# omuses/hqp

Hardware: AMD Instinct MI355X
Metric: KKT factor+solve/sec (fp64) (higher is better)
Workload: dtype f64; 1 GPU; C4 = BASELINE configs[3], the metric's 10^6-variable DOCP: multistage LQ optimal control QP, K=200 stages, nx=5000 states, nu=50 controls -> n=1015000 me=1005000 m=20000, dense fx/fu handed over as blocks, x_0 fixed, box bounds on u; plugin LQDOCP (STAGED engine), one system per GPU; stages=200, nx=5000, nu=50, n=1015000, me=1005000, m=20000, plugin=LQDOCP, kkt_dim_full=2040000

## Files before the change

### hqp_amd/csrc/hqpkkt.hip

```cpp
#include "hqpkkt_handle.hpp"

char g_last_hip_error[512] = "";
std::atomic<long long> g_live_bufs[2];

namespace kktdev {
__global__ void k_mfma_selftest(const double *A, const double *B, double *C) {
  const int lane = threadIdx.x & 63, lr = lane & 15, lk = lane >> 4;
  double4_t acc = {0.0, 0.0, 0.0, 0.0};
  for (int k0 = 0; k0 < 16; k0 += 4)
    acc = mfma_f64(A[lr * 16 + k0 + lk], B[(k0 + lk) * 16 + lr], acc);
  for (int rg = 0; rg < 4; rg++) C[(lk + 4 * rg) * 16 + lr] = acc[rg];
}
}

int hqpkkt_default_opts(hqpkkt_opts *o) {
  if (!o) return HQPKKT_E_NULL;
  std::memset(o, 0, sizeof(*o));
  o->mode = HQPKKT_MODE_FULL;
  o->device = 0;
  o->loc = HQPKKT_LOC_HOST;
  o->tol = 1.0;
  o->eps = 1e-10;
  o->pivot_eps = 1e-20;
  o->leaf_size = 0;
// ... 603 lines not shown
    case HQPKKT_E_SING: return "matrix is singular";
    case HQPKKT_E_FORMAT: return "CSR input not sorted / out of range";
    case HQPKKT_E_NULL: return "NULL objects passed";
    case HQPKKT_E_RANGE: return "parameter out of range";
    case HQPKKT_E_INTERN: return "call order violated";
    case HQPKKT_E_DEVICE: return g_last_hip_error[0] ? g_last_hip_error : "HIP device error";
    default: return "unknown status";
  }
}


int hqpkkt_debug_get(const hqpkkt_t *h, int what, int *out, long long *len) {
  if (!h || !len) return HQPKKT_E_NULL;
  if (!h->analyzed && what != 40) return HQPKKT_E_INTERN;
  const Analysis &an = h->an;
  const std::vector<int> *v = nullptr;
  std::vector<int> tmp;
  switch (what) {
    case 0: v = &an.q2e; break;
    case 1: v = &an.piv_start; break;
    case 2: v = &an.npiv; break;
    case 3: v = &an.nbor; break;
    case 4: v = &an.parent; break;
    case 5: v = &an.level; break;
    case 6:
      tmp.assign(an.bptr.begin(), an.bptr.end());
      v = &tmp;
      break;
    case 7: v = &an.bidx; break;
    case 8: v = &an.ent_er; break;
    case 9: v = &an.ent_ec; break;
    case 10: v = &an.node_owner; break;
    case 11: v = &an.xroots; break;
    case 20: case 21: case 22: case 23: case 24: case 25: case 26: case 27: case 28: case 32: case 33: case 34: case 35: case 36: case 37: case 38: case 39: case 41: case 42: case 43: case 44: case 45: case 46: case 47: {
      const int e = staged_debug_get(h, what, tmp);
      if (e) return e;
      v = &tmp;
      break;
    }
    case 30:
      tmp = {h->zd_used, h->zd_weak ? 1 : 0};
      v = &tmp;
      break;
    case 31:
      tmp = {h->top_n, h->top_n ? h->top_lt : h->an.nlevels, (int)h->top_lds, h->top_ns, h->small_tree ? 1 : 0, h->tree_factor ? 1 : 0, h->top_split ? 1 : 0};
      v = &tmp;
      break;
    case 40:
      tmp = {(int)g_live_bufs[0].load(), (int)g_live_bufs[1].load()};
      v = &tmp;
      break;
    default: return HQPKKT_E_RANGE;
  }
  *len = (long long)v->size();
  if (out && !v->empty()) std::memcpy(out, v->data(), sizeof(int) * v->size());
  return 0;
}

#ifdef HQPKKT_STAMPS
extern "C" int hqpkkt_debug_stamps(hqpkkt_t *h, int *out) {
  HIPCHK(hipDeviceSynchronize());
  HIPCHK(hipMemcpy(out, h->td.flags.p, sizeof(int) * 64, hipMemcpyDeviceToHost));
  return 0;
}
#endif

int hqpkkt_debug_read(hqpkkt_t *h, int what, int node, double *out, long long cap, long long *len) {
// ... 61 lines not shown
```

### hqp_amd/csrc/staged.hip.h

```cpp
#pragma once
#include <hip/hip_runtime.h>

#include <algorithm>

#include "staged_plan.hpp"
#include "staged_gemm.hip.h"

namespace stg {

struct HTerm {
  int s1, s2, wi;
};
__global__ void k_st_add_h(int nent, const long long *__restrict__ dst, const int *__restrict__ tptr,
                           const HTerm *__restrict__ terms, const double *__restrict__ vals,
                           const double *__restrict__ wt, double *__restrict__ G, int add) {
  const int e = blockIdx.x * blockDim.x + threadIdx.x;
  if (e >= nent) return;
  double s = 0.0;
  for (int k = tptr[e]; k < tptr[e + 1]; k++) s += vals[terms[k].s1] * vals[terms[k].s2] * wt[terms[k].wi];
  if (add)
    G[dst[e]] += s;
  else
    G[dst[e]] = s;
}
// ... 1647 lines not shown
};
__global__ void __launch_bounds__(256) k_st_fwd_small(FwdSmall a) {
  extern __shared__ __attribute__((aligned(16))) double sm[];
  const int tid = threadIdx.x, nt = blockDim.x;
  const int r = a.dyn[0], nl = a.dyn[1];
  const int *Rl = a.dyn + 2, *Ll = a.dyn + 2 + a.capn;
  const double *uy = a.uy;
  double *yN = sm;
  for (int i = tid; i < a.m; i += nt) a.u[i] = uy[i];
  for (int s = tid; s < r; s += nt) {
    double v = uy[a.m + s];
    for (int li = 0; li < nl; li++) v -= a.t[(long long)li * a.ldt + s] * a.eta[li];
    yN[Rl[s]] = v;
  }
  for (int li = tid; li < nl; li += nt) yN[Ll[li]] = a.eta[li];
  __syncthreads();
  const int c = r + nl;
  for (int i = tid; i < a.e; i += nt) a.dy[a.eq_rows[i]] = yN[i];
  for (int i = tid; i < a.cap_next; i += nt) a.eta_next[i] = (a.e + i < c) ? yN[a.e + i] : 0.0;
}

__global__ void k_st_x0_fixed(int n0, const int *__restrict__ fix_rows, const int *__restrict__ fix_src,
                              const double *__restrict__ vals, const double *__restrict__ r2, double *__restrict__ x0,
                              double *__restrict__ eta0, int cap0) {
  const int i = blockIdx.x * blockDim.x + threadIdx.x;
  if (i < n0) x0[i] = -r2[fix_rows[i]] / vals[fix_src[i]];
  if (i < cap0) eta0[i] = 0.0;
}
__global__ void k_st_y_fixed(int n0, const int *__restrict__ fix_rows, const int *__restrict__ fix_src,
                             const double *__restrict__ vals, const double *__restrict__ tmp, double *__restrict__ dy) {
  const int i = blockIdx.x * blockDim.x + threadIdx.x;
  if (i < n0) dy[fix_rows[i]] = -tmp[i] / vals[fix_src[i]];
}
__device__ void x0_lu_solve(const double *__restrict__ LU, long long ldq, const double *__restrict__ perm, int qmax, int q,
                            double *t, double *T) {
  const int tid = threadIdx.x, lane = tid & 63, wave = tid >> 6, nw = blockDim.x >> 6;
  if (tid == 0)
    for (int s = 0; s < q; s++) {
      const int r = (int)perm[qmax + s];
      const double x = t[s];
      t[s] = t[r], t[r] = x;
    }
  __syncthreads();
  for (int b0 = 0; b0 < q; b0 += 64) {
    const int nb = min(64, q - b0);
    for (int i = wave; i < nb; i += nw) {
      double sum = 0.0;
      for (int j = lane; j < b0; j += 64) sum += LU[(long long)(b0 + i) * ldq + j] * t[j];
      sum = kktdev::wave_sum(sum);
      if (lane == 0) t[b0 + i] -= sum;
    }
    for (int e = tid; e < nb * nb; e += blockDim.x) T[(e / nb) * 65 + e % nb] = LU[(long long)(b0 + e / nb) * ldq + b0 + e % nb];
    __syncthreads();
    if (wave == 0) {
      double y = lane < nb ? t[b0 + lane] : 0.0;
      for (int s = 0; s < nb; s++) {
        const double ys = __shfl(y, s);
        if (lane > s && lane < nb) y -= T[lane * 65 + s] * ys;
      }
      if (lane < nb) t[b0 + lane] = y;
    }
    __syncthreads();
  }
  for (int b0 = ((q - 1) / 64) * 64; b0 >= 0; b0 -= 64) {
    const int nb = min(64, q - b0);
    for (int i = wave; i < nb; i += nw) {
// ... 242 lines not shown
```

### hqp_amd/csrc/staged_engine.hip

```cpp
#include "hqpkkt_handle.hpp"

#include <algorithm>
#include <limits>

#include "staged.hip.h"
#include "staged_sparse.hip.h"
#include "staged_profile.hip.h"
#include "staged_rows.hip.h"
#include "staged_hess.hip.h"
#include "staged_host.hip.h"

static void staged_hess_symv(hqpkkt_t *h, StagedDev &d, const double *x, double *y) {
  const kktdev::StagedPlan &P = d.plan;
  if (d.hs_nz_max > 0 || !P.hess_packed) {
    const int nzmax = std::max(d.hs_nz_max, 1);
    KLAUNCH(h, KC_RESIDUAL, stg::k_hs_symv<<<dim3(std::min((nzmax + 3) / 4, 1024), P.K + 1), 256, 0, h->stream>>>(d.hess_desc.p, d.Qd.p, x, y));
  }
  if (d.hp_chunks_max > 0) {
    KLAUNCH(h, KC_RESIDUAL, stg::k_hp_symv_tiles<<<dim3(d.hp_chunks_max, P.K + 1), 256, 0, h->stream>>>(d.hp_desc.p, d.Qd.p, x, d.hess_scr.p));
    KLAUNCH(h, KC_RESIDUAL, stg::k_hp_symv_finish<<<dim3(d.hp_nt_max, P.K + 1), stg::HP_T, 0, h->stream>>>(d.hp_desc.p, d.hess_scr.p, y));
  }
}
int staged_dense_products(hqpkkt_t *h, const Vecs &v, const double **x1, const double **x2, int *ndyn, const double **xq) {
  StagedDev &d = *h->sd;
// ... 129 lines not shown
          for (long long c : {P.h_kept[k], P.h_cut[k]}) out.push_back((int)(unsigned)(c & 0xffffffffLL)), out.push_back((int)(c >> 32));
      }
      break;
    case 44:
      out.assign(P.K + 2, 0);
      if (h->sd->ctl.p) {
        unsigned w[3] = {0, 0, 0};
        if (hipDeviceSynchronize() != hipSuccess || hipMemcpy(w, h->sd->ctl.p, sizeof(w), hipMemcpyDeviceToHost) != hipSuccess) return HQPKKT_E_DEVICE;
        out[0] = (int)(w[1] + (w[2] ? 1 : 0));
      }
      for (size_t k = 0; k < h->sd->ctrl_rows.size() && k + 1 < out.size(); k++) out[k + 1] = h->sd->ctrl_rows[k];
      break;
    case 45:
      for (int k = 0; k <= P.K && P.hess_dense; k++) {
        out.push_back(P.hess_order(k)), out.push_back(P.ldQ[k]);
        out.push_back((int)(unsigned)(P.h_kept[k] & 0xffffffffLL)), out.push_back((int)(P.h_kept[k] >> 32));
      }
      break;
    case 47:
      for (int k = 0; k <= P.K && P.hess_packed; k++) {
        const int nz = P.hess_order(k);
        const bool pk = P.stage_packed(k);
        const long long nt = (nz + P.HESS_T - 1) / P.HESS_T, tiles = pk ? P.hess_tiles(nz) : 0;
        out.push_back(pk ? P.HESS_T : 0), out.push_back((int)tiles);
        for (long long c : {pk ? tiles * P.HESS_T * P.HESS_T : (long long)nz * P.ldQ[k], P.hess_handover(nz, pk), pk ? P.hess_slots(nt) * P.HESS_T : 0LL})
          out.push_back((int)(unsigned)(c & 0xffffffffLL)), out.push_back((int)(c >> 32));
      }
      break;
    case 46:
      if (!P.wr_rows.empty()) {
        out.push_back(P.rows_vec() ? 1 : 0), out.push_back((int)P.wr_rows.size());
        for (long long c : {P.c_kept, P.c_cut}) out.push_back((int)(unsigned)(c & 0xffffffffLL)), out.push_back((int)(c >> 32));
      }
      break;
    case 38:
      for (const GemmCache::Entry &t : h->sd->gemms.entries) {
        if (!t.s.cut()) continue;
        const int row[3] = {(int)t.s.f.tiles, (int)t.s.nslab, t.s.f.kind + (t.s.seg ? 100 : 0)};
        size_t q = 0;
        while (q < out.size() && !std::equal(row, row + 3, out.begin() + q)) q += 5;
        if (q == out.size()) out.insert(out.end(), {row[0], row[1], row[2], t.s.list, 0});
        out[q + 4] += t.hits;
      }
      break;
    default: return HQPKKT_E_RANGE;
  }
  return 0;
}

extern "C" {

int hqpkkt_set_dynamics_form(hqpkkt_t *h, int form) {
  return guarded([&]() -> int {
    if (!h) return HQPKKT_E_NULL;
    if (h->opts.mode != HQPKKT_MODE_STAGED) return HQPKKT_E_INTERN;
    if (form != HQPKKT_DYN_DENSE && form != HQPKKT_DYN_SPARSE && form != HQPKKT_DYN_PROFILE) return HQPKKT_E_RANGE;
    if (!h->sd) h->sd.reset(new StagedDev);
    h->sd->plan.want_sparse = form == HQPKKT_DYN_SPARSE;
    h->sd->plan.want_profile = form == HQPKKT_DYN_PROFILE;
    return 0;
  });
}

int hqpkkt_set_dense_columns(hqpkkt_t *h, int min_entries) {
  return guarded([&]() -> int {
    if (!h) return HQPKKT_E_NULL;
// ... 383 lines not shown
      KLAUNCH(h, KC_ASSEMBLE, stg::k_hu_update<<<dim3((unsigned)units_max, (unsigned)K1), 256, 0, h->stream>>>(d.hu_desc.p, d.Qd.p, V));
      HIPCHK(hipGetLastError());
      if (h->opts.loc != HQPKKT_LOC_DEVICE) HIPCHK(hipStreamSynchronize(h->stream));
    }
    if ((int)d.hess_set.size() != K1) d.hess_set.assign(K1, 0);
    for (int k = 0; k < K1; k++)
      if (hd[k].mode == 0) d.hess_set[k] = 1;
    h->factored = false;
    return 0;
  });
}

int hqpkkt_debug_stage_ranks(hqpkkt_t *h, int *out, int cap) {
  if (!h || !out) return HQPKKT_E_NULL;
  if (!h->sd || !h->uploaded) return HQPKKT_E_INTERN;
  HIPCHK(hipSetDevice(h->opts.device));
  HIPCHK(hipStreamSynchronize(h->stream));
  const kktdev::StagedPlan &P = h->sd->plan;
  for (int k = 0; k <= P.K && 2 * k + 1 < cap; k++)
    HIPCHK(hipMemcpy(out + 2 * k, h->sd->dyn.p + P.dyn_off[k], 2 * sizeof(int), hipMemcpyDeviceToHost));
  return 0;
}

int hqpkkt_debug_stage_block(hqpkkt_t *h, int k, double *out, long long cap, long long *len) {
  if (!h || !len) return HQPKKT_E_NULL;
  if (!h->sd || !h->uploaded || h->sd->plan.sharded) return HQPKKT_E_INTERN;
  const kktdev::StagedPlan &P = h->sd->plan;
  if (k < 0 || k > P.K) return HQPKKT_E_RANGE;
  const long long n = P.nk[k];
  *len = n * n;
  if (!out) return 0;
  if (cap < n * n) return HQPKKT_E_SIZES;
  HIPCHK(hipSetDevice(h->opts.device));
  HIPCHK(hipStreamSynchronize(h->stream));
  if (n) HIPCHK(hipMemcpy2D(out, sizeof(double) * n, h->sd->V.p + P.oV[k], sizeof(double) * P.ldv[k], sizeof(double) * n, n, hipMemcpyDeviceToHost));
  return 0;
}

namespace {
__global__ void k_fill_rand(double *p, long long n, unsigned long long seed) {
  long long i = (long long)blockIdx.x * blockDim.x + threadIdx.x;
  if (i >= n) return;
  unsigned long long x = (unsigned long long)i * 0x9E3779B97F4A7C15ULL + seed;
  x ^= x >> 30, x *= 0xBF58476D1CE4E5B9ULL, x ^= x >> 27, x *= 0x94D049BB133111EBULL, x ^= x >> 31;
  p[i] = (double)(x >> 11) * (1.0 / 9007199254740992.0) - 0.5;
}
__global__ void k_gemm_check(stg::GemmArgs g, int nsample, double *err) {
  const int sidx = blockIdx.x * blockDim.x + threadIdx.x;
  if (sidx >= nsample) return;
  unsigned long long x = (unsigned long long)sidx * 0x9E3779B97F4A7C15ULL + 12345;
  x ^= x >> 29, x *= 0xBF58476D1CE4E5B9ULL, x ^= x >> 32;
  int i = (int)(x % (unsigned long long)g.M), j = (int)((x >> 20) % (unsigned long long)g.N);
  int ci = i, cj = j;
  if (g.lower && i < j) {
    const int t = i;
    i = j, j = t;
    if (!g.mirror) ci = i, cj = j;
  }
  double s = 0.0, sa = 0.0;
  for (int k = 0; k < g.K; k++) {
    const double a = g.A[(long long)k * g.lda + i], b = g.B[(long long)k * g.ldb + j];
    s += a * b, sa += fabs(a * b);
  }
  for (int k = 0; k < g.K2; k++) {
    const double a = g.A2[(long long)k * g.lda2 + i], b = g.B2[(long long)k * g.ldb2 + j];
    s += a * b, sa += fabs(a * b);
// ... 778 lines not shown
```

### hqp_amd/csrc/staged_host.hip.h

```cpp
#pragma once

struct GemmCache {
  struct Entry {
    stg::GemmRequest rq;
    stg::GemmSchedule s;
    DBuf<stg::SkUnit> units;
    DBuf<int> order;
    int hits = 0;
  };
  std::vector<Entry> entries;
  Entry *find(const stg::GemmRequest &rq) {
    for (Entry &e : entries)
      if (e.rq == rq) return &e;
    return nullptr;
  }
  int get(const stg::GemmCaps &caps, const stg::GemmRequest &rq, bool create, Entry &local, Entry *&out) {
    if ((out = find(rq))) return 0;
    if (stg::gemm_schedule(caps, rq, local.s) != stg::GEMM_SCHED_OK) return HQPKKT_E_INTERN;
    out = &local;
    if (!local.s.kept()) return 0;
    if (!create) return HQPKKT_E_INTERN;
    local.rq = rq;
    if ((!local.s.tab.units.empty() && local.units.upload(local.s.tab.units)) || (!local.s.order.empty() && local.order.upload(local.s.order))) return HQPKKT_E_MEM;
    entries.push_back(std::move(local));
// ... 38 lines not shown
  DBuf<stg::StripTab> wtabs;
  DBuf<stg::RectTab> rtabs;
  DBuf<int> gtile;
  DBuf<unsigned> gowned;
  std::vector<long long> gowned_off;
  DBuf<stg::PackRect> prects;
  std::vector<int> prect_ptr;
  DBuf<stg::DynLoc> dyn_loc;
  DBuf<double> dyn_sum;
  long long dyn_sum_x2 = 0;
  StreamOwner stream_x;
  EventOwner ev_x1, ev_w[3], ev_x[3];
  struct SymvGroup {
    int first, count, tiles, fins;
    int kfirst, klast;
  };
  DBuf<stg::SymvItem> symv_items[2];
  std::vector<SymvGroup> symv_groups[2];
  std::vector<int> symv_rows_stage[2];
  DBuf<double> zeros;
  stg::GemmCaps caps;
  GemmCache gemms;
  DBuf<double> ks_ws2;
  DBuf<double> sk_ws;
  DBuf<unsigned> sk_cnt;
  StreamOwner stream2;
  EventOwner ev_fork, ev_join;
  bool overlap = false;
  int overlap_mode = 0;
  std::vector<char> fused;
  DBuf<double> fv_nrm;
  DBuf<unsigned> ctl;
  std::vector<char> ctrl_rows;
  DBuf<int> pf_rng;
  DBuf<double> pf_part;
  DBuf<stg::PackPanel> pk_tab;
  DBuf<double> pk_part;
  size_t lds_small = 0, lds_small_big = 0, lds_init = 0, lds_x0 = 0;
};

namespace {

bool env_no_symv() { static const bool v = getenv("HQPKKT_NO_SYMV") != nullptr; return v; }
int env_symv_from() { static const int v = getenv("HQPKKT_SYMV_FROM") ? atoi(getenv("HQPKKT_SYMV_FROM")) : 2048; return v; }
double env_block_gj_tol() { static const double v = getenv("HQPKKT_BLOCK_GJ_TOL") ? atof(getenv("HQPKKT_BLOCK_GJ_TOL")) : 1e-6; return v; }
bool env_spd_test_fail() { static const bool v = getenv("HQPKKT_SPD_TEST_FAIL") != nullptr; return v; }
struct StreamGuard {
  hqpkkt_t *h;
  hipStream_t s;
  ~StreamGuard() { h->stream = s; }
};
int stream_after(hqpkkt_t *h, hipEvent_t ev, hipStream_t from, hipStream_t to) {
  if (h->listing || from == to) return 0;
  HIPCHK(hipEventRecord(ev, from));
  HIPCHK(hipStreamWaitEvent(to, ev, 0));
  return 0;
}
struct StreamFork {
  hqpkkt_t *h;
  hipStream_t a, b;
  hipEvent_t ev_fork, ev_join;
  bool forked = false;
  int fork() {
    if (int e = stream_after(h, ev_fork, a, b)) return e;
    forked = true;
    return 0;
  }
  int join() {
    forked = false;
    return stream_after(h, ev_join, b, a);
  }
  ~StreamFork() {
    if (forked) (void)join();
  }
};

struct StagePtr {
  double *F, *V, *Y, *Rm, *Kinv, *Kmat, *N, *BT, *T, *v, *beta, *eta, *rho;
  int *dyn;
// ... 264 lines not shown
static void st_bwd_small(hqpkkt_t *h, StagedDev &d, int k, const StagePtr &sp, const StagePtr &sn, const double *r2, const double *gam) {
  const kktdev::StagedPlan &P = d.plan;
  stg::BwdSmall ba{P.nk[k], P.mk[k], P.nk[k + 1], P.eq_ptr[k + 1] - P.eq_ptr[k], P.capn[k], P.cap[k], P.qmax[k], d.eq_rows.p + P.eq_ptr[k], r2,
                   P.cap[k + 1] > 0 ? sn.dyn + 1 : nullptr, sn.beta, sn.BT, P.ldb[k + 1], r2 + P.nks[k], gam, sp.Kinv, sp.Kmat, P.ldq[k], sp.T, P.ldt[k],
                   sp.dyn, sp.rho, sp.beta};
  KLAUNCH(h, KC_ST_SMALL, stg::k_st_bwd_small<<<1, 256, sizeof(double) * (P.capn[k] + 3 * P.qmax[k] + 4 + 256), h->stream>>>(ba));
}
static int st_initial_state(hqpkkt_t *h, StagedDev &d, const double *r2) {
  const kktdev::StagedPlan &P = d.plan;
  hipStream_t s = h->stream;
  double *M = d.misc.p, *S = M + P.oS;
  const StagePtr s0 = stage_ptr(d, 0);
  const int n0 = P.nk[0];
  if (P.fixed_x0) {
    KLAUNCH(h, KC_ST_VEC, stg::k_st_x0_fixed<<<nblk(std::max(n0, P.cap[0])), 256, 0, s>>>(n0, d.fix_rows.p, d.fix_src.p, h->td.vals.p, r2, S,
                                                                                       s0.eta, P.cap[0]));
    return 0;
  }
  if (P.big0) {
    const int q = P.q0max, l8 = (q + 7) / 8 * 8;
    double *vec = M + P.oK0s + 3 * (long long)q + 8, *nb = vec, *pb = vec + l8, *y = vec + 2 * l8, *r = vec + 3 * l8;
    const stg::X0Vec xv{n0, P.cap[0], q, s0.dyn, M + P.oK0s, s0.v, s0.beta, nb, pb, pb, S, s0.eta};
    int e;
    KLAUNCH(h, KC_ST_VEC, stg::k_x0_rhs<<<nblk(q), 256, 0, s>>>(xv));
    if ((e = st_gemv_rows(h, stg::GemvRows{M + P.oK0, P.ldq0, q, q, nb, nullptr, nullptr, 0, nullptr, nullptr, y, 1.0})) ||
        (e = st_gemv_rows(h, stg::GemvRows{M + P.oK0m, P.ldq0, q, q, y, pb, nullptr, 0, nullptr, nullptr, r, -1.0})) ||
        (e = st_gemv_rows(h, stg::GemvRows{M + P.oK0, P.ldq0, q, q, r, y, nullptr, 0, nullptr, nullptr, pb, 1.0})))
      return e;
    KLAUNCH(h, KC_ST_VEC, stg::k_x0_out<<<nblk(n0 + P.cap[0]), 256, 0, s>>>(xv));
  }
  KLAUNCH(h, KC_ST_SMALL, stg::k_st_x0_free<<<1, 256, d.lds_x0, s>>>(n0, P.cap[0], P.q0max, M + P.oK0, M + P.oK0m, M + P.oK0s, P.ldq0, s0.dyn, s0.v,
                                                            s0.beta, S, s0.eta));
  return 0;
}
static void st_fwd_small(hqpkkt_t *h, StagedDev &d, int k, const StagePtr &sp, const StagePtr &sn, double *dy) {
  const kktdev::StagedPlan &P = d.plan;
  hipStream_t s = h->stream;
  const int nn = P.nk[k];
  double *xk = d.misc.p + P.oS + P.nmk[k], *uy = d.misc.p + P.oUy;
  if (P.qmax[k] > 0) {
    const stg::GemvRows gr{sp.Rm, P.ldy[k], P.qmax[k], nn, xk, sp.rho, nullptr, 0, nullptr, nullptr, uy, -1.0};
    stg::gemv_launch_wide(gr, s, [&](auto &&launch) { KLAUNCH(h, KC_ST_VEC, launch()); });
  }
  stg::FwdSmall fa{nn, P.mk[k], P.eq_ptr[k + 1] - P.eq_ptr[k], P.capn[k], P.cap[k], P.qmax[k], uy, sp.T, P.ldt[k],
                   sp.dyn, sp.eta, d.eq_rows.p + P.eq_ptr[k], xk + nn, dy, sn.eta, P.cap[k + 1]};
  KLAUNCH(h, KC_ST_SMALL, stg::k_st_fwd_small<<<1, 256, sizeof(double) * (P.capn[k] + 4), s>>>(fa));
}

int staged_analyze(hqpkkt_t *h, int n, int me, int m, bool dense_dyn) {
  if (!h->sd) h->sd.reset(new StagedDev);
  StagedDev &d = *h->sd;
  kktdev::StagedPlan &P = d.plan;
  std::vector<int> gnx = P.given_nx, gnu = P.given_nu;
  const bool want_sparse = P.want_sparse, want_profile = P.want_profile;
  const int want_heavy = P.want_heavy, want_rows = P.want_rows;
  const bool want_packed = P.want_packed, want_hess_dense = P.want_hess_dense, want_hess_packed = P.want_hess_packed;
  P = kktdev::StagedPlan();
  P.given_nx = gnx, P.given_nu = gnu, P.want_sparse = want_sparse, P.want_profile = want_profile, P.want_heavy = want_heavy, P.want_packed = want_packed, P.want_rows = want_rows;
  P.want_hess_dense = want_hess_dense, P.want_hess_packed = want_hess_packed;
  P.dense_dyn = dense_dyn;
  if (h->shard_count > 16) return HQPKKT_E_RANGE;
  P.shard_rank = h->shard_rank, P.shard_count = h->shard_count;
  P.sharded = h->shard_count > 1 || h->xchg_fn || h->xchg_sfn;
  if ((want_sparse || want_profile) && dense_dyn) return HQPKKT_E_INTERN;
  if ((want_sparse || want_profile) && P.sharded) return HQPKKT_E_RANGE;
  if (want_hess_dense && P.sharded) return HQPKKT_E_RANGE;
// ... 235 lines not shown
    d.fused.assign(P.K + 1, 0);
    long long nrm = 0;
    std::vector<std::pair<stg::GemmRequest, stg::GemmSchedule>> asked;
    auto ask = [&](const stg::GemmRequest &rq) -> const stg::GemmSchedule & {
      for (const auto &a : asked)
        if (a.first == rq) return a.second;
      asked.emplace_back(rq, stg::GemmSchedule{});
      if (stg::gemm_schedule(d.caps, rq, asked.back().second)) asked.back().second = stg::GemmSchedule{};
      return asked.back().second;
    };
    if (mode != 0 && !P.sharded && !P.sparse_dyn && d.zeros.p)
      for (int k = 0; k < P.K; k++) {
        const int nn = P.nk[k], q = P.qmax[k], np = P.nk[k + 1];
        if (P.profile_dyn && P.pf_stage[k]) continue;
        if (P.wide_count(k)) continue;
        if (P.big[k] || q <= 0 || q > 64 || (nn & 1) || np <= 0) continue;
        stg::GemmRequest rt;
        rt.M = P.mk[k], rt.N = nn + P.mk[k], rt.K = np;
        if (ask(stg::gemm_request(staged_v_args(d, k))).f.kind == stg::GEMM_FORM_NONE) continue;
        d.ctrl_rows[k] = ask(rt).f.kind == stg::GEMM_FORM_KS && ask(stg::gemm_request(staged_w_args(d, k, true))).seg;
        if (mode != 1 && (!d.ctrl_rows[k] || (nn >= 1280 && nn <= 4096))) {
          d.ctrl_rows[k] = 0;
          continue;
        }
        d.fused[k] = 1;
        nrm = std::max(nrm, (long long)q * P.ldy[k]);
      }
    d.fv_nrm.release();
    if (nrm > 0) {
      if ((e = d.fv_nrm.alloc((size_t)nrm + 8192))) return e;
      HIPCHK(hipMemset(d.fv_nrm.p, 0, sizeof(double) * ((size_t)nrm + 8192)));
    }
  }
  if (P.sharded) {
    const int NR = P.shard_count, RK = P.shard_rank;
    std::vector<stg::StripTab> wt(P.K + 1);
    std::vector<stg::RectTab> rt(P.K + 1);
    std::vector<stg::PackRect> pr;
    d.prect_ptr.assign(P.K + 1, 0);
    for (int k = 0; k < P.K; k++) {
      const int *cut = &P.xcut[(size_t)k * (NR + 1)];
      stg::StripTab &t = wt[k];
      stg::RectTab &r = rt[k];
      t.nranks = r.nranks = NR;
      for (int p = 0; p <= NR; p++) {
        t.cut[p] = r.cut[p] = cut[p];
        if (p < NR) t.off[p] = (long long)p * P.fgslot[k], t.ld[p] = (cut[p + 1] - cut[p] + P.mk[k] + 7) / 8 * 8;
      }
      for (auto &b : r.blk) b.off[0] = b.off[1] = 0, b.rsplit = 1 << 30, b.pad = 0;
      d.prect_ptr[k] = (int)pr.size();
      for (int q = P.xrect_ptr[k]; q < P.xrect_ptr[k + 1]; q++) {
        const kktdev::StagedPlan::XRect &x = P.xrects[q];
        stg::RectTab::Block &b = r.blk[x.a * 16 + x.b];
        const long long off = (long long)x.owner * P.xslot[k] + x.off;
        if (x.r0 == cut[x.a])
          b.off[0] = off;
        else
          b.off[1] = off, b.rsplit = x.r0;
        if (x.owner == RK) {
          stg::PackRect pk{};
          if (x.mine_rows)
            pk.r0 = x.r0, pk.c0 = x.c0, pk.rows = x.r1 - x.r0, pk.cols = x.c1 - x.c0, pk.transpose = 0;
          else
            pk.r0 = x.c0, pk.c0 = x.r0, pk.rows = x.c1 - x.c0, pk.cols = x.r1 - x.r0, pk.transpose = 1;
          pk.off = x.off;
          pr.push_back(pk);
// ... 248 lines not shown
  gu.rects = d.rtabs.p + k;
  if ((e = st_gemm(h, gu, KC_ST_GEMM_UPD))) return e;
  st_keep_rows(h, d, k);
  return 0;
}


static int staged_stage_fused(hqpkkt_t *h, int k) {
  StagedDev &d = *h->sd;
  const kktdev::StagedPlan &P = d.plan;
  StagePtr sp = stage_ptr(d, k), sn = stage_ptr(d, k + 1);
  const int nn = P.nk[k], mm = P.mk[k], np = P.nk[k + 1], nz = nn + mm;
  const long long ldf = P.ldf[k], ldg = P.ldg[k];
  double *G = d.misc.p + P.oG, *W = d.misc.p + P.oW, *nRm = d.fv_nrm.p;
  const int ne_x = P.h_mid[k] - P.h_ptr[k], ne_u = P.h_ptr[k + 1] - P.h_mid[k];
  int e;
  const bool seg = d.ctrl_rows[k];
  if ((e = st_gemm(h, staged_w_args(d, k, seg)))) return e;
  stg::GemmArgs gu{W + nn, ldf, sp.F, ldf, nullptr, 0, G + nn * ldg, ldg, mm, nz, np, 1.0, 0.0, 0, 0};
  if (seg) gu.guard = d.ctl.p + 2;
  if (mm > 0 && (e = st_gemm(h, gu, KC_ST_GEMM_UPD))) return e;
  if (seg && !h->listing) KLAUNCH(h, KC_ST_SMALL, stg::k_ctrl_rows_end<<<1, 64, 0, h->stream>>>(d.ctl.p));
  st_add_q(h, d, k, nn, nz, nz, 0, G, ldg);
  st_add_h(h, d, P.h_mid[k], ne_u, G);
  if ((e = st_carried_rows(h, d, k, sp, sn, true)) || (e = st_eliminate(h, d, k, sp, sn, G, true, nRm))) return e;
  if ((e = st_gemm(h, staged_v_args(d, k)))) return e;
  st_add_q(h, d, k, 0, nn, nn, 0, sp.V, P.ldv[k]);
  if (ne_x)
    KLAUNCH(h, KC_ASSEMBLE, stg::k_st_add_h_sym<<<nblk(ne_x), 256, 0, h->stream>>>(ne_x, d.h_dst.p + P.h_ptr[k], d.h_tptr.p + P.h_ptr[k], d.h_terms.p,
                                                                                 h->td.vals.p, h->td.wt.p, sp.V, ldg, P.ldv[k]));
  return 0;
}

static int staged_stage_dense(hqpkkt_t *h, int k) {
  StagedDev &d = *h->sd;
  const kktdev::StagedPlan &P = d.plan;
  StagePtr sp = stage_ptr(d, k), sn = stage_ptr(d, k + 1);
  const int nn = P.nk[k], mm = P.mk[k], np = P.nk[k + 1], nz = nn + mm;
  const long long ldf = P.ldf[k], ldg = P.ldg[k], ldvn = P.ldv[k + 1];
  double *G = d.misc.p + P.oG, *W = d.misc.p + P.oW;
  const bool ovl = d.overlap && mm > 0 && (nn % 2 == 0) && (d.overlap_mode == 1 || (nn >= 1280 && nn <= 4096)) && !P.wide_count(k);
  hipStream_t sA = h->stream, sB = ovl ? d.stream2 : h->stream;
  StreamGuard guard{h, sA};
  StreamFork chain{h, sA, sB, d.ev_fork, d.ev_join};
  const int ne_x = P.h_mid[k] - P.h_ptr[k], ne_u = P.h_ptr[k + 1] - P.h_mid[k];
  int e;
  if ((e = st_gemm(h, stg::GemmArgs{sn.V, ldvn, sp.F, ldf, nullptr, 0, W, ldf, np, nz, np, 1.0, 0.0, 0, 0})) || (e = chain.fork())) return e;
  if (!ovl) {
    if ((e = st_gemm(h, stg::GemmArgs{sp.F, ldf, W, ldf, nullptr, 0, G, ldg, nz, nz, np, 1.0, 0.0, 1, 0}))) return e;
    st_add_q(h, d, k, 0, nz, nz, 1, G, ldg);
    st_add_h(h, d, P.h_ptr[k], ne_x + ne_u, G);
    if ((e = st_add_h_wide(h, d, k, G, ldg))) return e;
  } else {
    if ((e = st_gemm(h, stg::GemmArgs{sp.F, ldf, W, ldf, nullptr, 0, G, ldg, nn, nn, np, 1.0, 0.0, 1, 0}))) return e;
    st_add_q(h, d, k, 0, nn, nn, 1, G, ldg);
    st_add_h(h, d, P.h_ptr[k], ne_x, G);
    h->stream = sB;
    if ((e = st_gemm(h, stg::GemmArgs{W + nn, ldf, sp.F, ldf, nullptr, 0, G + nn * ldg, ldg, mm, nz, np, 1.0, 0.0, 0, 0}, KC_ST_GEMM, false))) return e;
    st_add_q(h, d, k, nn, nz, nz, 0, G, ldg);
    st_add_h(h, d, P.h_mid[k], ne_u, G);
  }
  h->stream = sB;
  if ((e = st_carried_rows(h, d, k, sp, sn, !ovl)) || (e = st_eliminate(h, d, k, sp, sn, G, !ovl))) return e;
  h->stream = sA;
  if ((e = chain.join())) return e;
  return st_gemm(h, stg::GemmArgs{sp.Y, P.ldy[k], sp.Rm, P.ldy[k], G, ldg, sp.V, P.ldv[k], nn, nn, P.qmax[k], -1.0, 1.0, 1, 1}, KC_ST_GEMM_UPD);
// ... 68 lines not shown
  st_add_q(h, d, k, 0, nz, nz, 0, G, ldg);
  st_add_h(h, d, P.h_ptr[k], P.h_ptr[k + 1] - P.h_ptr[k], G);
  if ((e = st_add_h_wide(h, d, k, G, ldg)) || (e = st_eliminate(h, d, k, sp, sn, G, true))) return e;
  return st_gemm(h, stg::GemmArgs{sp.Y, P.ldy[k], sp.Rm, P.ldy[k], G, P.ldg[k], sp.V, P.ldv[k], nn, nn, P.qmax[k], -1.0, 1.0, 1, 1}, KC_ST_GEMM_UPD);
}

static int staged_run_factor(hqpkkt_t *h, const double *z, const double *w) {
  Analysis &an = h->an;
  StagedDev &d = *h->sd;
  kktdev::StagedPlan &P = d.plan;
  hipStream_t s = h->stream;
  const int m = an.m, K = P.K;
  const bool timed = !h->capturing && !h->listing;
  int e;
  if (!h->listing) {
    const long long vk = (long long)P.nk[K] * P.ldv[K];
    kktdev::k_clear<<<(int)std::max<long long>(1, std::min<long long>(4096, (vk / 2 + 1023) / 1024)), 256, 0, s>>>(stage_ptr(d, K).V, vk, h->td.flags.p);
  }
  if (timed) HIPCHK(hipEventRecord(h->ev0, s));
  if (m > 0) KLAUNCH(h, KC_ASSEMBLE, k_weights<<<nblk(m), 256, 0, s>>>(1, m, an.n + an.me, z, w, h->td.wt.p, nullptr, h->td.flags.p));
  if (timed) HIPCHK(hipEventRecord(h->ev1, s));
  {
    StagePtr sp = stage_ptr(d, K);
    const int nK = P.nk[K], eK = P.eq_ptr[K + 1] - P.eq_ptr[K];
    st_add_q(h, d, K, 0, nK, nK, 0, sp.V, P.ldv[K]);
    st_add_h(h, d, P.h_ptr[K], P.h_ptr[K + 1] - P.h_ptr[K], sp.V, P.hess_dense ? 1 : 0);
    if (!P.sharded && (e = st_add_h_wide(h, d, K, sp.V, P.ldv[K]))) return e;
    KLAUNCH(h, KC_ST_SMALL, stg::k_st_last<<<nblk(std::max(nK, 1)), 256, 0, s>>>(nK, eK, P.cap[K], sp.N, P.ldn[K], sp.BT, P.ldb[K], sp.dyn));
    if (P.sharded) st_keep_rows(h, d, K);
  }
  if (P.sharded && K > 0 && (e = staged_gather_f(h, K - 1))) return e;
  for (int k = K - 1; k >= 0; k--)
    if ((e = P.sharded                            ? staged_stage_sharded(h, k)
             : P.sparse_dyn                       ? staged_stage_sparse(h, k)
             : P.profile_dyn && P.pf_stage[k]     ? staged_stage_profile(h, k)
             : d.fused[k]                         ? staged_stage_fused(h, k)
                                                  : staged_stage_dense(h, k)))
      return e;
  {
    StagePtr s0 = stage_ptr(d, 0);
    if (P.fixed_x0)
      KLAUNCH(h, KC_ST_SMALL, stg::k_st_check_fixed<<<1, 64, 0, s>>>(s0.dyn, h->td.flags.p));
    else if (P.big0) {
      double *scr = d.misc.p + P.oScr;
      const int q = P.q0max;
      const stg::X0Args xa{P.nk[0], q, s0.V, P.ldv[0], s0.BT, P.ldb[0], s0.dyn, d.misc.p + P.oK0, d.misc.p + P.oK0m, d.misc.p + P.oK0s,
                           P.ldq0, scr, h->td.flags.p};
      KLAUNCH(h, KC_ST_SMALL, stg::k_x0_prepare<<<nblk((long long)q * q), 256, 0, s>>>(xa));
      if ((e = st_blk_sweep(h, scr, q, true))) return e;
      KLAUNCH(h, KC_ST_SMALL, stg::k_x0_final<<<nblk((long long)q * q), 256, 0, s>>>(xa));
      const stg::BigScratch bs = stg::big_scratch(scr, q);
      if ((e = st_gemm(h, stg::GemmArgs{xa.K0mat, P.ldq0, xa.K0inv, P.ldq0, nullptr, 0, bs.Ks, bs.ldk, q, q, q, 1.0, 0.0, 0, 0}, KC_ST_GEMM_UPD, true)))
        return e;
      KLAUNCH(h, KC_ST_SMALL, stg::k_x0_check<<<1, 1024, 0, s>>>(xa, env_block_gj_tol()));
      KLAUNCH(h, KC_ST_SMALL, stg::k_st_init_factor<1024><<<1, 1024, d.lds_init, s>>>(P.nk[0], P.cap[0], s0.V, P.ldv[0], s0.BT, P.ldb[0], s0.dyn,
                                                                                    d.misc.p + P.oK0, d.misc.p + P.oK0m, d.misc.p + P.oK0s, P.ldq0, P.q0max, h->td.flags.p,
                                                                                    scr, bs.flags));
    } else
      KLAUNCH(h, KC_ST_SMALL, stg::k_st_init_factor<256><<<1, 256, d.lds_init, s>>>(P.nk[0], P.cap[0], s0.V, P.ldv[0], s0.BT, P.ldb[0], s0.dyn,
                                                                                  d.misc.p + P.oK0, d.misc.p + P.oK0m, d.misc.p + P.oK0s, P.ldq0, P.q0max, h->td.flags.p, nullptr, nullptr));
  }
  if (timed) HIPCHK(hipEventRecord(h->evs1, s));
  if (!h->listing) HIPCHK(hipGetLastError());
  return 0;
}

// ... 86 lines not shown
                          [&](auto &&launch) { KLAUNCH(h, KC_ST_VEC, launch()); });
      continue;
    }
    if (!sh) {
      if ((e = st_gemv_rows(h, stg::GemvRows{sp.F, P.ldf[k], np, nn + mm, xk, v.r2 + P.nks[k], nullptr, 0, nullptr, nullptr, S + P.nmk[k + 1], 1.0})))
        return e;
      continue;
    }
    if ((e = st_gemv_rows(h, stg::GemvRows{sp.F, P.ldfl[k], np, wd, xk + c0, nullptr, nullptr, 0, nullptr, nullptr, xp + (long long)RK * P.xpslot, 1.0})))
      return e;
    if ((e = exchange(h, HQPKKT_XCHG_ALLGATHER, xp, P.xpslot, NR, nullptr))) return e;
    if ((e = st_gemv_rows(h, stg::GemvRows{sp.F + wd, P.ldfl[k], np, mm, xk + nn, v.r2 + P.nks[k], nullptr, 0, nullptr, nullptr, tt, 1.0}))) return e;
    KLAUNCH(h, KC_ST_VEC, stg::k_st_sum_slots<<<nblk(np), 256, 0, s>>>(np, NR, xp, P.xpslot, tt, S + P.nmk[k + 1]));
    if (wdn > 0 &&
        (e = st_gemv_rows(h, stg::GemvRows{sn.Vs, P.ldv[k + 1], wdn, np, S + P.nmk[k + 1], sn.v + c0n,
                                           P.cap[k + 1] > 0 ? sn.BT + (long long)c0n * P.ldb[k + 1] : nullptr, P.ldb[k + 1], sn.dyn + 1, sn.eta,
                                           dyx + P.nks[k] + c0n, 1.0})))
      return e;
  }
  if (!sh) {
    for (int gi = 0; gi < (int)d.symv_groups[1].size(); gi++)
      if ((e = staged_symv_group(h, d, 1, gi, nullptr, v.dy))) return e;
    if ((e = staged_symv_rows(h, d, 1, nullptr, v.dy))) return e;
  }
  StagePtr sK = stage_ptr(d, K), s0 = stage_ptr(d, 0);
  const int eK = P.eq_ptr[K + 1] - P.eq_ptr[K], n0 = P.nk[0];
  if (eK) KLAUNCH(h, KC_ST_VEC, stg::k_st_y_last<<<nblk(eK), 256, 0, s>>>(eK, d.eq_rows.p + P.eq_ptr[K], sK.eta, v.dy));
  if (sh) {
    if (P.fixed_x0 && width(0) > 0 &&
        (e = st_gemv_rows(h, stg::GemvRows{s0.Vs, P.ldv[0], width(0), n0, S, s0.v + cut0(0), nullptr, 0, nullptr, nullptr, dyx + P.ndyn + cut0(0), 1.0})))
      return e;
    if (ndx > 0 && (e = exchange(h, HQPKKT_XCHG_ALLREDUCE_SUM, dyx, ndx, 1, nullptr))) return e;
    if (P.ndyn > 0) KLAUNCH(h, KC_ST_VEC, stg::k_st_copy<<<nblk(P.ndyn), 256, 0, s>>>(P.ndyn, dyx, v.dy));
  } else if (P.fixed_x0 && (e = st_symv(h, d, stg::GemvRows{s0.V, P.ldv[0], n0, n0, S, s0.v, nullptr, 0, nullptr, nullptr, tmp, 1.0})))
    return e;
  if (P.fixed_x0) KLAUNCH(h, KC_ST_VEC, stg::k_st_y_fixed<<<nblk(n0), 256, 0, s>>>(n0, d.fix_rows.p, d.fix_src.p, h->td.vals.p, sh ? dyx + P.ndyn : tmp, v.dy));
  KLAUNCH(h, KC_VECTOR, stg::k_st_negate<<<nblk(n), 256, 0, s>>>(n, S, v.dx));
  if (m > 0)
    KLAUNCH(h, KC_VECTOR, k_red_dzdw<<<nblk(m), 256, 0, s>>>(m, C.ptr.p, C.col.p, C.src.p, h->td.vals.p, v.dx, h->td.wt.p, h->td.tz.p, v.r3, v.dz, v.dw));
  if (wide) st_rows_rows(h, d, stg::RowsGemv{nullptr, nullptr, 0, nullptr, nullptr, v.dx, h->td.tz.p, h->td.wt.p, v.r3, v.dz, v.dw, nullptr});
  HIPCHK(hipGetLastError());
  return 0;
}
```

### hqp_amd/csrc/staged_plan.cpp

```cpp
#include "staged_plan.hpp"

#include <algorithm>
#include <cstdint>
#include <numeric>

namespace kktdev {

namespace {
const int CARRY_MAX = 256;
const int CONTROLS_MAX = 512;
inline int up8(long long x) { return (int)((x + 7) / 8 * 8); }
inline long long up16(long long x) { return (x + 15) / 16 * 16; }
}

int stages_from_staircase(int n, int rows, const int *row_len, const int *last_col, const int *prev_col,
                          std::vector<int> &states, std::vector<int> &controls, std::vector<int> &first_col, int &dyn_rows) {
  struct Stage {
    int first_target;
    int produced;
  };
  std::vector<Stage> found;
  int target = -1;
  dyn_rows = -1;
  for (int i = 0; i < rows && dyn_rows < 0; i++) {
// ... 539 lines not shown
        h_tptr.push_back(h_tptr.back());
        h_ptr[(int)(e.key >> 45) + 1]++;
        if (!((e.key >> 44) & 1)) nstate[(int)(e.key >> 45)]++;
        prev = e.key;
      }
      h_terms.push_back(e.t);
      h_tptr.back()++;
    }
    for (int k = 0; k <= K; k++) h_ptr[k + 1] += h_ptr[k];
    h_mid.assign(K + 1, 0);
    for (int k = 0; k <= K; k++) h_mid[k] = h_ptr[k] + nstate[k];
  }

  flops_factor = 0, bytes_step = 0;
  for (int k = 0; k < K; k++) {
    const long long nn = nk[k], mm = mk[k], np = nk[k + 1], nz = nn + mm, q = qmax[k];
    if (sparse_dyn) {
      const long long nd = heavy_count(k), nnz = sp_nnz[k] - hv_nnz[k];
      flops_factor += 2 * nnz * np + nnz * nz + 2 * nnz * cap[k + 1];
      flops_factor += 2 * np * np * nd + 2 * np * nd * nd + 2 * (long long)cap[k + 1] * np * nd + 2 * nnz * nd;
      bytes_step += 8 * (2 * np * np + 4 * (long long)sp_nnz[k] + 2 * q * nn);
    } else {
      flops_factor += 2 * np * np * nz;
      flops_factor += np * nz * nz;
      flops_factor += 2 * (long long)cap[k + 1] * np * nz;
      bytes_step += 8 * (2 * np * np + 2 * np * nz + 2 * q * nn);
    }
    flops_factor += 2 * q * q * nn + q * nn * nn;
  }
  for (int k = 0; k <= K; k++) {
    const long long nz = k < K ? nk[k] + mk[k] : nk[k];
    flops_factor += wide_count(k) * nz * nz;
  }
  return 0;
}

void StagedPlan::narrow_copies(const int *Cp, const int *Ci, const int *Cs, const int *CTp, const int *CTi, const int *CTs) {
  cn = Narrow(), ctn = Narrow(), c_kept = c_cut = 0;
  if (wr_rows.empty()) return;
  std::vector<char> is_wide(m, 0);
  for (int r : wr_rows) is_wide[r] = 1;
  cn.ptr.assign(m + 1, 0), ctn.ptr.assign(n + 1, 0);
  for (int r = 0; r < m; r++) {
    for (int p = Cp[r]; p < Cp[r + 1] && !is_wide[r]; p++) cn.col.push_back(Ci[p]), cn.src.push_back(Cs[p]);
    cn.ptr[r + 1] = (int)cn.col.size();
  }
  for (int c = 0; c < n; c++) {
    for (int p = CTp[c]; p < CTp[c + 1]; p++)
      if (!is_wide[CTi[p]]) ctn.col.push_back(CTi[p]), ctn.src.push_back(CTs[p]);
    ctn.ptr[c + 1] = (int)ctn.col.size();
  }
  c_kept = (long long)cn.col.size(), c_cut = (long long)Cp[m] - c_kept;
}

}
```

### hqp_amd/csrc/staged_plan.hpp

```cpp
#pragma once
#include <algorithm>
#include <cstddef>
#include <vector>

namespace kktdev {

inline long long gj_lds_bytes(long long q) {
  const long long cv = q > 64 ? q : 64, rv = q > 128 ? q : 128;
  return q * (q | 1) * 8 + (q + cv + rv) * 8 + 3 * q * 4 + 64;
}

int stages_from_staircase(int n, int rows, const int *row_len, const int *last_col, const int *prev_col,
                          std::vector<int> &states, std::vector<int> &controls, std::vector<int> &first_col, int &dyn_rows);

struct StagedPlan {
  int n = 0, me = 0, m = 0, K = 0;
  int nq = 0, na = 0, nc = 0;
  std::vector<int> nk, mk, nmk;
  std::vector<int> nks;
  int ndyn = 0;
  std::vector<int> eq_ptr, eq_rows;
  bool fixed_x0 = false;
  std::vector<int> fix_rows, fix_src;
  bool dense_dyn = false;
// ... 64 lines not shown

  std::vector<int> cap, capn, qmax;
  int q0max = 0, ldq0 = 8;
  std::vector<char> big;
  int big0 = 0;
  long long scratch_elems = 0, oScr = 0;

  std::vector<int> ldf, ldv, ldy, ldn, ldb, ldq, ldt, ldg;
  std::vector<long long> oF, oV;
  std::vector<long long> oY, oR, oK, oKm, oN, oBT, oT;
  std::vector<long long> oVec;
  long long oW = 0, oG = 0, oK0 = 0, oK0m = 0, oK0s = 0, oRes = 0, oGam = 0, oTT = 0, oPart = 0, oS = 0, oQv = 0, oTmp = 0, oUy = 0, oSym = 0;
  long long oGv = 0, oSymB = 0, symb_elems = 0;
  static long long symv_need(long long N) { return ((N + 63) / 64 + (N + 511) / 512) * (N + 8); }
  long long f_elems = 0, v_elems = 0, misc_elems = 0;
  int part_chunks = 1;
  std::vector<int> dyn_off;
  int dyn_ints = 0;

  struct Term {
    int s1, s2, wi;
  };
  std::vector<int> h_ptr, h_tptr;
  std::vector<int> h_mid;
  std::vector<long long> h_dst;
  std::vector<Term> h_terms;

  std::vector<long long> a_dst;
  std::vector<int> chk_idx, chk_kind;

  long long flops_factor = 0;
  long long bytes_step = 0;

  int shard_rank = 0, shard_count = 1;
  bool sharded = false;
  std::vector<int> xcut;
  std::vector<int> xw;
  std::vector<int> ldfl;
  std::vector<long long> oFl, oVs;
  long long oVf[2] = {0, 0};
  long long oFg[2] = {0, 0};
  std::vector<long long> fgslot;
  long long oWl = 0, oWu = 0;
  std::vector<int> ldwl;
  int ldwu = 8;
  long long oX = 0;
  std::vector<long long> xslot;
  long long oXV = 0;
  long long xvslot = 0;
  long long oXP = 0;
  long long xpslot = 0;
  long long oDyx = 0;
  struct XRect {
    int a, b;
    int r0, r1, c0, c1;
    int owner;
    bool mine_rows;
    long long off;
  };
  std::vector<XRect> xrects;
  std::vector<int> xrect_ptr;
  std::vector<int> gtile;
  std::vector<int> gtile_ptr;

  std::vector<int> given_nx, given_nu;

// ... 6 lines not shown
```

Baseline: 0.8460 KKT factor+solve/s.

## Skip forming stage-0 state block when x0 is fixed, apply it matrix-free

When x_0 is fixed, the stage-0 factorisation no longer builds the full nn x nn state block of the value matrix. It computes only the control rows and columns (V1*Fu, then G rows for the controls) and eliminates from those. The solve then applies the missing state block matrix-free: a new warp-per-row Hessian-term kernel plus gemv/symv through F, V1 and Y/Rm. The full block is recomputed lazily only if a caller asks for V[0] after factoring. This removes the large nx^2 * nx GEMMs at stage 0 in exchange for extra gemvs in every solve. It is gated by an env default and a set of plan conditions.

```diff
diff --git a/hqp_amd/csrc/hqpkkt.hip b/hqp_amd/csrc/hqpkkt.hip
--- a/hqp_amd/csrc/hqpkkt.hip
+++ b/hqp_amd/csrc/hqpkkt.hip
@@ -659,7 +659,7 @@
     case 9: v = &an.ent_ec; break;
     case 10: v = &an.node_owner; break;
     case 11: v = &an.xroots; break;
-    case 20: case 21: case 22: case 23: case 24: case 25: case 26: case 27: case 28: case 32: case 33: case 34: case 35: case 36: case 37: case 38: case 39: case 41: case 42: case 43: case 44: case 45: case 46: case 47: {
+    case 20: case 21: case 22: case 23: case 24: case 25: case 26: case 27: case 28: case 32: case 33: case 34: case 35: case 36: case 37: case 38: case 39: case 41: case 42: case 43: case 44: case 45: case 46: case 47: case 48: {
       const int e = staged_debug_get(h, what, tmp);
       if (e) return e;
       v = &tmp;
diff --git a/hqp_amd/csrc/staged.hip.h b/hqp_amd/csrc/staged.hip.h
--- a/hqp_amd/csrc/staged.hip.h
+++ b/hqp_amd/csrc/staged.hip.h
@@ -1703,6 +1703,34 @@
   const int i = blockIdx.x * blockDim.x + threadIdx.x;
   if (i < n0) dy[fix_rows[i]] = -tmp[i] / vals[fix_src[i]];
 }
+__global__ void __launch_bounds__(256) k_st_hxx_vec(int n, int nent, const long long *__restrict__ dst, const int *__restrict__ tptr,
+                                                    const HTerm *__restrict__ terms, const double *__restrict__ vals,
+                                                    const double *__restrict__ wt, long long ld, const double *__restrict__ x,
+                                                    const double *__restrict__ add, double *__restrict__ y) {
+  const int lane = threadIdx.x & 63, i = blockIdx.x * 4 + (threadIdx.x >> 6);
+  if (i >= n) return;
+  const long long row0 = (long long)i * ld;
+  auto first_from = [&](long long key) {
+    int lo = 0, hi = nent;
+    while (lo < hi) {
+      const int mid = (lo + hi) >> 1;
+      if (dst[mid] < key)
+        lo = mid + 1;
+      else
+        hi = mid;
+    }
+    return lo;
+  };
+  const int e0 = first_from(row0), e1 = first_from(row0 + ld);
+  double s = 0.0;
+  for (int e = e0 + lane; e < e1; e += 64) {
+    double v = 0.0;
+    for (int k = tptr[e]; k < tptr[e + 1]; k++) v += vals[terms[k].s1] * vals[terms[k].s2] * wt[terms[k].wi];
+    s += v * x[dst[e] - row0];
+  }
+  s = kktdev::wave_sum(s);
+  if (lane == 0) y[i] = add[i] + s;
+}
 __device__ void x0_lu_solve(const double *__restrict__ LU, long long ldq, const double *__restrict__ perm, int qmax, int q,
                             double *t, double *T) {
   const int tid = threadIdx.x, lane = tid & 63, wave = tid >> 6, nw = blockDim.x >> 6;
diff --git a/hqp_amd/csrc/staged_engine.hip b/hqp_amd/csrc/staged_engine.hip
--- a/hqp_amd/csrc/staged_engine.hip
+++ b/hqp_amd/csrc/staged_engine.hip
@@ -185,6 +185,9 @@
         out.push_back(P.rows_vec() ? 1 : 0), out.push_back((int)P.wr_rows.size());
         for (long long c : {P.c_kept, P.c_cut}) out.push_back((int)(unsigned)(c & 0xffffffffLL)), out.push_back((int)(c >> 32));
       }
+      break;
+    case 48:
+      out = {(h->uploaded ? h->sd->first_fixed : P.first_fixed_ok && (end_stages_from_env() & 1)) ? 1 : 0, 0, 0};
       break;
     case 38:
       for (const GemmCache::Entry &t : h->sd->gemms.entries) {
@@ -634,6 +637,8 @@
   if (!out) return 0;
   if (cap < n * n) return HQPKKT_E_SIZES;
   HIPCHK(hipSetDevice(h->opts.device));
+  if (k == 0 && h->factored)
+    if (int e = staged_first_block(h)) return e;
   HIPCHK(hipStreamSynchronize(h->stream));
   if (n) HIPCHK(hipMemcpy2D(out, sizeof(double) * n, h->sd->V.p + P.oV[k], sizeof(double) * P.ldv[k], sizeof(double) * n, n, hipMemcpyDeviceToHost));
   return 0;
diff --git a/hqp_amd/csrc/staged_host.hip.h b/hqp_amd/csrc/staged_host.hip.h
--- a/hqp_amd/csrc/staged_host.hip.h
+++ b/hqp_amd/csrc/staged_host.hip.h
@@ -94,6 +94,7 @@
   DBuf<double> fv_nrm;
   DBuf<unsigned> ctl;
   std::vector<char> ctrl_rows;
+  bool first_fixed = false;
   DBuf<int> pf_rng;
   DBuf<double> pf_part;
   DBuf<stg::PackPanel> pk_tab;
@@ -107,6 +108,10 @@
 int env_symv_from() { static const int v = getenv("HQPKKT_SYMV_FROM") ? atoi(getenv("HQPKKT_SYMV_FROM")) : 2048; return v; }
 double env_block_gj_tol() { static const double v = getenv("HQPKKT_BLOCK_GJ_TOL") ? atof(getenv("HQPKKT_BLOCK_GJ_TOL")) : 1e-6; return v; }
 bool env_spd_test_fail() { static const bool v = getenv("HQPKKT_SPD_TEST_FAIL") != nullptr; return v; }
+int end_stages_from_env() {
+  const char *s = getenv("HQPKKT_END_STAGES");
+  return s ? atoi(s) : 3;
+}
 struct StreamGuard {
   hqpkkt_t *h;
   hipStream_t s;
@@ -437,6 +442,26 @@
   KLAUNCH(h, KC_ST_SMALL, stg::k_st_x0_free<<<1, 256, d.lds_x0, s>>>(n0, P.cap[0], P.q0max, M + P.oK0, M + P.oK0m, M + P.oK0s, P.ldq0, s0.dyn, s0.v,
                                                             s0.beta, S, s0.eta));
   return 0;
+}
+static int st_first_fixed_vec(hqpkkt_t *h, StagedDev &d, double *tmp) {
+  const kktdev::StagedPlan &P = d.plan;
+  double *M = d.misc.p, *S = M + P.oS, *gam = M + P.oGam, *tt = M + P.oTT, *uy = M + P.oUy;
+  const StagePtr sp = stage_ptr(d, 0), sn = stage_ptr(d, 1);
+  const int nn = P.nk[0], np = P.nk[1], q = P.qmax[0];
+  int e;
+  if (P.hess_dense && (e = st_gemv_rows(h, stg::GemvRows{d.Qd.p + P.oQ[0], P.ldQ[0], nn, nn, S, sp.v, nullptr, 0, nullptr, nullptr, gam, 1.0}))) return e;
+  KLAUNCH(h, KC_ST_VEC, stg::k_st_hxx_vec<<<(nn + 3) / 4, 256, 0, h->stream>>>(nn, P.h_mid[0] - P.h_ptr[0], d.h_dst.p + P.h_ptr[0], d.h_tptr.p + P.h_ptr[0],
+                                                                          d.h_terms.p, h->td.vals.p, h->td.wt.p, P.ldg[0], S, P.hess_dense ? gam : sp.v, tmp));
+  if ((e = st_gemv_rows(h, stg::GemvRows{sp.F, P.ldf[0], np, nn, S, nullptr, nullptr, 0, nullptr, nullptr, tt, 1.0})) ||
+      (e = st_symv(h, d, stg::GemvRows{sn.V, P.ldv[1], np, np, tt, nullptr, nullptr, 0, nullptr, nullptr, gam, 1.0})) ||
+      (e = st_gemv_cols(h, d, sp.F, P.ldf[0], np, nn, gam, tmp, 1.0, tt)))
+    return e;
+  if (q <= 0) {
+    KLAUNCH(h, KC_ST_VEC, stg::k_st_copy<<<nblk(nn), 256, 0, h->stream>>>(nn, tt, tmp));
+    return 0;
+  }
+  if ((e = st_gemv_rows(h, stg::GemvRows{sp.Rm, P.ldy[0], q, nn, S, nullptr, nullptr, 0, nullptr, nullptr, uy, 1.0}))) return e;
+  return st_gemv_cols(h, d, sp.Y, P.ldy[0], q, nn, uy, tt, -1.0, tmp);
 }
 static void st_fwd_small(hqpkkt_t *h, StagedDev &d, int k, const StagePtr &sp, const StagePtr &sn, double *dy) {
   const kktdev::StagedPlan &P = d.plan;
@@ -738,6 +763,8 @@
       HIPCHK(hipMemset(d.fv_nrm.p, 0, sizeof(double) * ((size_t)nrm + 8192)));
     }
   }
+  d.first_fixed = P.first_fixed_ok && (end_stages_from_env() & 1);
+  h->st.flops_factor = P.flops_factor - (d.first_fixed ? P.flops_first_fixed : 0);
   if (P.sharded) {
     const int NR = P.shard_count, RK = P.shard_rank;
     std::vector<stg::StripTab> wt(P.K + 1);
@@ -1052,6 +1079,48 @@
   return 0;
 }
 
+static int staged_stage_first_fixed(hqpkkt_t *h) {
+  StagedDev &d = *h->sd;
+  const kktdev::StagedPlan &P = d.plan;
+  StagePtr sp = stage_ptr(d, 0), sn = stage_ptr(d, 1);
+  const int nn = P.nk[0], mm = P.mk[0], np = P.nk[1], nz = nn + mm;
+  const long long ldf = P.ldf[0], ldg = P.ldg[0];
+  double *G = d.misc.p + P.oG, *W = d.misc.p + P.oW;
+  int e;
+  if ((e = st_gemm(h, stg::GemmArgs{sn.V, P.ldv[1], sp.F + nn, ldf, nullptr, 0, W + nn, ldf, np, mm, np, 1.0, 0.0, 0, 0}, KC_ST_GEMM_UPD)) ||
+      (e = st_gemm(h, stg::GemmArgs{W + nn, ldf, sp.F, ldf, nullptr, 0, G + nn * ldg, ldg, mm, nz, np, 1.0, 0.0, 0, 0}, KC_ST_GEMM_UPD)))
+    return e;
+  st_add_q(h, d, 0, nn, nz, nz, 0, G, ldg);
+  st_add_h(h, d, P.h_mid[0], P.h_ptr[1] - P.h_mid[0], G);
+  if ((e = st_carried_rows(h, d, 0, sp, sn, true))) return e;
+  return st_eliminate(h, d, 0, sp, sn, G, true);
+}
+static int staged_first_block(hqpkkt_t *h) {
+  StagedDev &d = *h->sd;
+  const kktdev::StagedPlan &P = d.plan;
+  if (!d.first_fixed) return 0;
+  StagePtr sp = stage_ptr(d, 0), sn = stage_ptr(d, 1);
+  const int nn = P.nk[0], mm = P.mk[0], np = P.nk[1];
+  const long long ldf = P.ldf[0], ldg = P.ldg[0];
+  double *G = d.misc.p + P.oG, *W = d.misc.p + P.oW;
+  struct Listing {
+    hqpkkt_t *h;
+    ~Listing() { h->listing = false; }
+  } walk{h};
+  for (int pass = 0; pass < 2; pass++) {
+    int e;
+    h->listing = pass == 0;
+    if ((e = st_gemm(h, stg::GemmArgs{sn.V, P.ldv[1], sp.F, ldf, nullptr, 0, W, ldf, np, nn + mm, np, 1.0, 0.0, 0, 0})) ||
+        (e = st_gemm(h, stg::GemmArgs{sp.F, ldf, W, ldf, nullptr, 0, G, ldg, nn, nn, np, 1.0, 0.0, 1, 0})))
+      return e;
+    st_add_q(h, d, 0, 0, nn, nn, 1, G, ldg);
+    st_add_h(h, d, P.h_ptr[0], P.h_mid[0] - P.h_ptr[0], G);
+    if ((e = st_gemm(h, stg::GemmArgs{sp.Y, P.ldy[0], sp.Rm, P.ldy[0], G, ldg, sp.V, P.ldv[0], nn, nn, P.qmax[0], -1.0, 1.0, 1, 1}, KC_ST_GEMM_UPD))) return e;
+  }
+  HIPCHK(hipGetLastError());
+  return 0;
+}
+
 static int staged_stage_dense(hqpkkt_t *h, int k) {
   StagedDev &d = *h->sd;
   const kktdev::StagedPlan &P = d.plan;
@@ -1186,6 +1255,7 @@
   if (P.sharded && K > 0 && (e = staged_gather_f(h, K - 1))) return e;
   for (int k = K - 1; k >= 0; k--)
     if ((e = P.sharded                            ? staged_stage_sharded(h, k)
+             : k == 0 && d.first_fixed            ? staged_stage_first_fixed(h)
              : P.sparse_dyn                       ? staged_stage_sparse(h, k)
              : P.profile_dyn && P.pf_stage[k]     ? staged_stage_profile(h, k)
              : d.fused[k]                         ? staged_stage_fused(h, k)
@@ -1338,7 +1408,8 @@
       return e;
     if (ndx > 0 && (e = exchange(h, HQPKKT_XCHG_ALLREDUCE_SUM, dyx, ndx, 1, nullptr))) return e;
     if (P.ndyn > 0) KLAUNCH(h, KC_ST_VEC, stg::k_st_copy<<<nblk(P.ndyn), 256, 0, s>>>(P.ndyn, dyx, v.dy));
-  } else if (P.fixed_x0 && (e = st_symv(h, d, stg::GemvRows{s0.V, P.ldv[0], n0, n0, S, s0.v, nullptr, 0, nullptr, nullptr, tmp, 1.0})))
+  } else if (P.fixed_x0 && (e = d.first_fixed ? st_first_fixed_vec(h, d, tmp)
+                                             : st_symv(h, d, stg::GemvRows{s0.V, P.ldv[0], n0, n0, S, s0.v, nullptr, 0, nullptr, nullptr, tmp, 1.0})))
     return e;
   if (P.fixed_x0) KLAUNCH(h, KC_ST_VEC, stg::k_st_y_fixed<<<nblk(n0), 256, 0, s>>>(n0, d.fix_rows.p, d.fix_src.p, h->td.vals.p, sh ? dyx + P.ndyn : tmp, v.dy));
   KLAUNCH(h, KC_VECTOR, stg::k_st_negate<<<nblk(n), 256, 0, s>>>(n, S, v.dx));
diff --git a/hqp_amd/csrc/staged_plan.cpp b/hqp_amd/csrc/staged_plan.cpp
--- a/hqp_amd/csrc/staged_plan.cpp
+++ b/hqp_amd/csrc/staged_plan.cpp
@@ -595,6 +595,13 @@
     const long long nz = k < K ? nk[k] + mk[k] : nk[k];
     flops_factor += wide_count(k) * nz * nz;
   }
+  first_fixed_ok = fixed_x0 && !sharded && K >= 1 && !sparse_dyn && !(profile_dyn && pf_stage[0]) && wide_count(0) == 0 &&
+                   !(hess_dense && stage_packed(0)) && nk[0] % 2 == 0 && mk[0] > 0 && nk[1] > 0;
+  flops_first_fixed = 0;
+  if (first_fixed_ok) {
+    const long long nn = nk[0], mm = mk[0], np = nk[1], nz = nn + mm, q = qmax[0];
+    flops_first_fixed = 2 * np * np * nz + np * nz * nz + q * nn * nn - (2 * np * np * mm + 2 * np * mm * nz);
+  }
   return 0;
 }
 
diff --git a/hqp_amd/csrc/staged_plan.hpp b/hqp_amd/csrc/staged_plan.hpp
--- a/hqp_amd/csrc/staged_plan.hpp
+++ b/hqp_amd/csrc/staged_plan.hpp
@@ -120,6 +120,9 @@
   long long flops_factor = 0;
   long long bytes_step = 0;
 
+  bool first_fixed_ok = false;
+  long long flops_first_fixed = 0;
+
   int shard_rank = 0, shard_count = 1;
   bool sharded = false;
   std::vector<int> xcut;
```

Result: no change. 0.8498 KKT factor+solve/s, median of 6 (+0.5%).
